# Megvii-CSG/MegReader

Measured on AMD Instinct MI355X. Metric: training images/sec, CRNN-CTC 32x128 crops, batch 256 per GPU, higher is better.
Workload: dtype bf16; 1 GPU; CRNN + 1D-CTC training step (BASELINE.json configs[1]): 32x128 crops, T=33, C=38, Adam; global_batch=256, per_gpu_batch=256, parallelism=dp1, launch=hipGraph replay

## Files before the change

megreader_amd/_lib.py:

```python
import ctypes
import os
import re

import torch

_HERE = os.path.dirname(os.path.abspath(__file__))
LIB_PATH = os.environ.get("MEGREADER_HIP_LIB") or os.path.join(_HERE, "csrc", "libmegreader_hip.so")
HEADER_PATH = os.path.join(os.path.dirname(_HERE), "include", "megreader_hip.h")

MR_F32 = 0
MR_BF16 = 1

_PARAM_TYPES = {"int": ctypes.c_int, "long long": ctypes.c_longlong, "float": ctypes.c_float, "double": ctypes.c_double,
                "hipStream_t": ctypes.c_void_p}
_RETURN_TYPES = {"int": ctypes.c_int, "long long": ctypes.c_longlong, "const char*": ctypes.c_char_p}


def _ctype(decl, context, array_ok=False):
    m = re.fullmatch(r"(.*?)(\w+)(?:\[(\d+)\])?", decl.strip(), re.S)
    base = " ".join(m.group(1).split()) if m else ""
    ctype = ctypes.c_void_p if "*" in base else _PARAM_TYPES.get(base)
    if ctype is None or (m.group(3) and not array_ok):
        raise TypeError("cannot bind %r in `%s`: no ctypes mapping for that type" % (decl.strip(), " ".join(context.split())))
    return m.group(2), ctype * int(m.group(3)) if m.group(3) else ctype, base == "hipStream_t"
# ... 19 lines not shown
    for stmt in filter(None, (s.strip() for s in text.split(";"))):
        if stmt == "}":
            continue
        m = re.fullmatch(r"(.*?)\b(mr_\w+)\s*\((.*)\)", stmt, re.S)
        ret = re.sub(r"\s*\*\s*", "*", " ".join(m.group(1).split())) if m else None
        if ret not in _RETURN_TYPES or m.group(2) in functions:
            raise TypeError("cannot bind `%s`: not a declaration `int | long long | const char* mr_name(...)`"
                            % " ".join(stmt.split()))
        params = [] if m.group(3).strip() in ("", "void") else [_ctype(p, stmt) for p in m.group(3).split(",")]
        functions[m.group(2)] = (_RETURN_TYPES[ret], [p[1] for p in params], bool(params) and params[-1][2])
    return functions, structs, defines


def _read_header(path):
    if not os.path.exists(path):
        raise RuntimeError("C ABI header not found at %s -- the ctypes binding is derived from it (there is no fallback table)"
                           % path)
    with open(path) as f:
        return parse_header(f.read())


FUNCTIONS, STRUCTS, _DEFINES = _read_header(HEADER_PATH)
ABI_VERSION = _DEFINES["MR_ABI_VERSION"]
TUNING_FIELDS = tuple(name for name, _ in STRUCTS["mr_tuning"] if name != "reserved")
_STREAMED = frozenset(name for name, (_, _, streamed) in FUNCTIONS.items() if streamed)

_lib = None


class Tuning(ctypes.Structure):
    _fields_ = STRUCTS["mr_tuning"]


def get_tuning():
    t = Tuning()
    if load().mr_tuning_get(ctypes.byref(t)) != 0:
        raise RuntimeError("mr_tuning_get failed: %s" % load().mr_last_error().decode())
    return {name: getattr(t, name) for name in TUNING_FIELDS}


def set_tuning(**fields):
    lib = load()
    t = Tuning()
    if lib.mr_tuning_get(ctypes.byref(t)) != 0:
        raise RuntimeError("mr_tuning_get failed: %s" % lib.mr_last_error().decode())
    old = {}
    for name, value in fields.items():
        if name not in TUNING_FIELDS:
            raise KeyError("mr_tuning has no field %r" % name)
        old[name] = getattr(t, name)
        setattr(t, name, int(value))
    if lib.mr_tuning_set(ctypes.byref(t)) != 0:
        raise RuntimeError("mr_tuning_set failed: %s" % lib.mr_last_error().decode())
    return old


def _install_setter_shims(lib):
    def one(field, clamp=None):
        def setter(value):
            value = int(value)
            if clamp is not None and not clamp(value):
                return get_tuning()[field]
            return set_tuning(**{field: value})[field]
        return setter
    lib.mr_set_nt_variant = one("nt_variant", lambda v: v in (1, 2))
    lib.mr_set_nt_deep = one("nt_deep", lambda v: 0 <= v <= 2)
    lib.mr_set_nt_big = one("nt_big", lambda v: -1 <= v <= 13)
    lib.mr_set_nt_p8 = one("nt_p8")
    lib.mr_set_gemm_skinny = lambda v: one("gemm_skinny")(1 if v else 0)
    lib.mr_set_tn_big = one("tn_big", lambda v: -1 <= v <= 2)
    lib.mr_set_tn_buf = one("tn_buf", lambda v: v in (0, 1))
    lib.mr_set_tn_taps = one("tn_taps", lambda v: v in (0, 1))
    lib.mr_set_tn_taps_group = one("tn_taps_group", lambda v: v >= 0)
    lib.mr_set_tn_group = one("tn_group", lambda v: v >= 0)
    lib.mr_set_tn_fin = one("tn_fin", lambda v: v in (0, 2))
    lib.mr_set_tn_taps_fin = one("tn_taps_fin", lambda v: 0 <= v <= 2)
    lib.mr_set_tn_taps_w8 = one("tn_taps_w8", lambda v: v in (0, 1))
    lib.mr_set_tn_model = lambda v: one("tn_model")(1 if v else 0)
    lib.mr_set_tn_splits = lambda v: one("tn_splits")(max(0, int(v)))
    lib.mr_set_bn_fused = one("bn_fused", lambda v: v in (0, 1))
    lib.mr_set_dcn_fused = lambda v: one("dcn_fused")(1 if v else 0)
    lib.mr_set_dcn_v1_bwd = lambda v: one("dcn_v1_bwd")(1 if v else 0)

    def set_lstm_persist(on):
        set_tuning(lstm_persist=int(on) if int(on) in (0, 1, 2) else 1)
        return 0
    lib.mr_set_lstm_persist = set_lstm_persist

    def set_lstm_variant(fwd_bn, bwd_bn):
        f = {}
        if fwd_bn >= 0:
            f["lstm_fwd_bn"] = fwd_bn
        if bwd_bn >= 0:
            f["lstm_bwd_bn"] = bwd_bn
        set_tuning(**f)
        return 0
    lib.mr_set_lstm_variant = set_lstm_variant

    def force_nt_tile(bm, bn):
        set_tuning(nt_force_bm=bm, nt_force_bn=bn if bm else 0)
        return 0
    lib.mr_force_nt_tile = force_nt_tile


def header_symbols():
    return sorted(FUNCTIONS)


def _bind(lib, functions, optional=False):
    for name, (restype, argtypes, _) in functions.items():
        if optional and not hasattr(lib, name):
            continue
        fn = getattr(lib, name)
        fn.restype, fn.argtypes = restype, argtypes


def load():
    global _lib
    if _lib is not None:
        return _lib
    if not os.path.exists(LIB_PATH):
        raise RuntimeError(
            "libmegreader_hip.so not found at %s -- build it with `python -c 'import __graft_entry__ as g; "
            "g.build()'` or `make -C megreader_amd/csrc` (there is no CPU fallback)" % LIB_PATH)
    lib = ctypes.CDLL(LIB_PATH)
    if lib.mr_abi_version() != ABI_VERSION:
        raise RuntimeError("%s implements C ABI version %d, this binding expects %d -- rebuild it (`make -C megreader_amd/csrc`)"
                           % (LIB_PATH, lib.mr_abi_version(), ABI_VERSION))
    _bind(lib, FUNCTIONS)
    _bind(lib, _read_header(os.path.join(os.path.dirname(HEADER_PATH), "megreader_hip_ablation.h"))[0], optional=True)
    _install_setter_shims(lib)
    _lib = lib
    if torch.cuda.is_available():
        if lib.mr_init() != 0:
            raise RuntimeError("mr_init failed: %s" % lib.mr_last_error().decode())
    elif lib.mr_init() != 0:
        err = lib.mr_last_error().decode()
        if "MEGREADER_TUNING" in err:
            raise RuntimeError("mr_init failed: %s" % err)
    return lib


def dtype_code(dtype):
    if dtype == torch.float32:
        return MR_F32
    if dtype == torch.bfloat16:
        return MR_BF16
    raise TypeError("megreader_amd kernels support float32 and bfloat16, got %s" % dtype)


def vec_of(dtype):
    return 4 if dtype == torch.float32 else 8


def stream_ptr():
    return torch.cuda.current_stream().cuda_stream


def ptr(t):
    return 0 if t is None else t.data_ptr()


class KernelTimer(object):

    def __init__(self, names, track_deferred=False):
        self.names = set(names)
# ... 97 lines not shown
```

megreader_amd/csrc/gemm_conv.hip:

```cpp
#include "igemm_core.h"
#include "igemm_p8.h"
#include "tn_taps.h"
#include "nt32.h"
#include "device.h"
#include "../../include/megreader_hip.h"

#include <algorithm>
#include <cmath>
#include <map>
#include <mutex>
#include <vector>

namespace mr {

static bool aligned16(const void* p) { return (((uintptr_t)p) & 15) == 0; }

#define g_nt_variant MR_TUNE(nt_variant)
#define g_nt_deep MR_TUNE(nt_deep)

struct BnbRequest { const void* x; const void* y; const float* mean; const float* rstd; };
struct NtEpilogue {
  const float* bias = nullptr;
  int relu = 0;
  const void* addend = nullptr;
// ... 87 lines not shown
  if constexpr (AMODE != 1) {
    if (g_nt_variant == 2 && nt_fits_buffer<T>(a, g, AMODE)) {
      const int grid = cdiv(cdiv(a.M - a.m_begin, BM), 8) * 8 * cdiv(a.N, BN);
      NtArgs a2 = a;
      a2.zero = zero_page();
      if (!a2.zero) { set_error("zero page allocation failed"); return MR_ERR_LAUNCH; }
      if constexpr (AMODE == 2) {
        if (o.bnb.x != nullptr) {
          EpiStoreB<T> eb;
          static_cast<EpiStore<T>&>(eb) = epi;
          eb.bnb_x = (const T*)o.bnb.x;
          eb.bnb_y = (const T*)o.bnb.y;
          eb.bnb_mean = o.bnb.mean;
          eb.bnb_rstd = o.bnb.rstd;
          return launch_nt_glds<T, BM, BN, AMODE, EpiStoreB<T>>(a2, g, eb, grid, tiles, stream);
        }
      }
      return launch_nt_glds<T, BM, BN, AMODE, EpiStore<T>>(a2, g, epi, grid, tiles, stream);
    }
  }
  if (a.m_begin != 0) { set_error("row-range launches need the direct-to-LDS NT kernel"); return MR_ERR_ARG; }
  if (o.stats) o.stats_missed = true;
  epi.stats = nullptr;
  hipLaunchKernelGGL((igemm_nt_kernel<T, BM, BN, AMODE, EpiStore<T>>), dim3(tiles), dim3(256), 0, stream, a, g,
                     epi);
  MR_CHECK_LAUNCH();
  return MR_OK;
}

#define g_big_mode MR_TUNE(nt_big)
#ifdef MR_ABLATION
static int g_tn_abl = 0;
#endif
#define g_tn_model MR_TUNE(tn_model)
#define g_tn_splits MR_TUNE(tn_splits)
#define g_tn_buf MR_TUNE(tn_buf)
#define g_tn_taps MR_TUNE(tn_taps)
#define g_tn_group MR_TUNE(tn_group)
#define g_tn_fin MR_TUNE(tn_fin)
#define g_tn_big MR_TUNE(tn_big)

static int nt_big_choice(int M, int N, int K) {
  if (g_big_mode < 0) return 0;
  if (g_big_mode > 0) return g_big_mode;
  if (N % 256 != 0 || K < MR_TUNE(nt_big_min_k)) return 0;
  const int cus = num_cus();
  const long long tiles = (long long)cdiv(M, 256) * (N / 256);
  const long long rounds = (tiles + cus - 1) / cus;
  const double util = (double)M * N / ((double)rounds * cus * 256 * 256);
  if (util >= 0.85) return 1;
  const long long tiles272 = (long long)cdiv(M, 272) * (N / 256);
  const long long rounds272 = (tiles272 + cus - 1) / cus;
  const double util272 = (double)M * N / ((double)rounds272 * cus * 272 * 256);
  if (util272 >= 0.85) {
    const int tiles_n = N / 256;
    double alt = 1e300;
    if (cus % tiles_n == 0) {
      const long long rows_per_round = (long long)(cus / tiles_n) * 256;
      const long long head = (M / rows_per_round) * rows_per_round;
      if (head > 0 && (M - head) * 8 <= M) alt = (double)(head / rows_per_round) * 256 + (head == M ? 0 : 57);
    }
    if ((double)rounds272 * 272 < alt) return 3;
  }
  return 0;
}

static long long nt_head_rows(int M, int N, int K) {
  if (g_big_mode != 0 || N % 256 != 0 || K < MR_TUNE(nt_big_min_k)) return 0;
  const int cus = num_cus();
  const int tiles_n = N / 256;
  if (cus % tiles_n != 0) return 0;
  const long long rows_per_round = (long long)(cus / tiles_n) * 256;
  const long long head = (M / rows_per_round) * rows_per_round;
  return (head > 0 && (M - head) * 8 <= M) ? head : 0;
}

template <typename T, int WM, int WN, int TM, int TN, int AMODE>
static int launch_nt_big(const NtArgs& a, const ConvGeom& g, void* C, long long ldc, NtEpilogue& o, hipStream_t stream) {
  constexpr int BM = WM * TM * 16, BN = WN * TN * 16;
  const EpiStore<T> epi = make_epi_store<T>(C, ldc, a.M, a.N, o);
  NtArgs a2 = a;
  a2.zero = zero_page();
  if (!a2.zero) { set_error("zero page allocation failed"); return MR_ERR_LAUNCH; }
  constexpr size_t lds = 2 * (size_t)(BM + BN) * 128;
  auto kern = igemm_nt_big_kernel<T, WM, WN, TM, TN, AMODE, EpiStore<T>>;
  if (const int rc = ensure_dynamic_lds(kern, lds)) return rc;
  const int tiles_m = cdiv(a.M - a.m_begin, BM), tiles_n = cdiv(a.N, BN);
  const int grid = cdiv(tiles_m, 8) * 8 * tiles_n;
  hipLaunchKernelGGL(kern, dim3(grid), dim3(64 * WM * WN), lds, stream, a2, g, epi);
  MR_CHECK_LAUNCH();
  return MR_OK;
}

#define g_use_p8 MR_TUNE(nt_p8)
template <typename T, int AMODE>
static int launch_nt_p8(const NtArgs& a, const ConvGeom& g, void* C, long long ldc, NtEpilogue& o, hipStream_t stream) {
  if constexpr (sizeof(T) != 2) {
    return launch_nt_big<T, 2, 4, 8, 4, AMODE>(a, g, C, ldc, o, stream);
  } else {
    if (!g_use_p8) return launch_nt_big<T, 2, 4, 8, 4, AMODE>(a, g, C, ldc, o, stream);
    const EpiStore<T> epi = make_epi_store<T>(C, ldc, a.M, a.N, o);
    NtArgs a2 = a;
    a2.zero = zero_page();
    if (!a2.zero) { set_error("zero page allocation failed"); return MR_ERR_LAUNCH; }
    constexpr size_t lds = 2 * (size_t)(256 + 256) * 128;
    const int tiles_m = cdiv(a.M - a.m_begin, 256), tiles_n = cdiv(a.N, 256);
    const int grid = cdiv(tiles_m, 8) * 8 * tiles_n;
#define MR_P8_LAUNCH(ABL_)                                                    \
  {                                                                           \
    auto kern = igemm_nt_p8_kernel<AMODE, EpiStore<T>, ABL_>;                 \
    if (const int rc = ensure_dynamic_lds(kern, lds)) return rc;              \
    hipLaunchKernelGGL(kern, dim3(grid), dim3(512), lds, stream, a2, g, epi); \
  }
#ifdef MR_ABLATION
    if (g_use_p8 == 2) MR_P8_LAUNCH(1)
    else if (g_use_p8 == 3) MR_P8_LAUNCH(2)
    else if (g_use_p8 == 4) MR_P8_LAUNCH(3)
    else
#endif
    MR_P8_LAUNCH(0)
#undef MR_P8_LAUNCH
    MR_CHECK_LAUNCH();
    return MR_OK;
  }
}

struct TileChoice { int bm, bn; };
static inline TileChoice forced_tile() { return TileChoice{MR_TUNE(nt_force_bm), MR_TUNE(nt_force_bn)}; }
static TileChoice nt_tile(int M, int N) {
  if (forced_tile().bm) return forced_tile();
  static const int bms[3] = {128, 96, 64};
  static const int bns[2] = {128, 64};
  auto eff = [](int bm, int bn) {
    if (bn == 128) return bm == 128 ? 1.0 : bm == 96 ? 0.90 : 0.85;
    return bm == 128 ? 0.60 : bm == 96 ? 0.60 : 0.55;
  };
  const int cus = num_cus();
  TileChoice best = {128, 128};
  double best_t = 1e300;
  for (int i = 0; i < 3; ++i)
    for (int j = 0; j < 2; ++j) {
      const int bm = bms[i], bn = bns[j];
      if (bn == 128 && N <= 64) continue;
      const long long tiles = (long long)cdiv(M, bm) * cdiv(N, bn);
      const int lds = 2 * (bm + bn) * 128;
      int per_cu = (160 * 1024) / lds;
      if (per_cu > 3) per_cu = 3;
      long long c = (tiles + cus - 1) / cus;
      if (c > per_cu) c = per_cu;
      const long long rounds = (tiles + cus * c - 1) / (cus * c);
      const double t = (double)rounds * c * bm * bn / eff(bm, bn);
      if (t < best_t) { best_t = t; best.bm = bm; best.bn = bn; }
    }
  return best;
}

static bool nt_use_288x128(int M, int N, int K) {
  if (g_big_mode != 0 || N % 128 != 0 || K < 2048) return false;
  const int cus = num_cus();
  const long long tiles = (long long)cdiv(M, 288) * (N / 128);
  const long long rounds = (tiles + cus - 1) / cus;
  const double util = (double)M * N / ((double)rounds * cus * 288 * 128);
  if (util < 0.85) return false;
  const TileChoice t = nt_tile(M, N);
  const long long t4 = (long long)cdiv(M, t.bm) * cdiv(N, t.bn);
  int per_cu = (160 * 1024) / (2 * (t.bm + t.bn) * 128);
// ... 378 lines not shown
        void* ws = nullptr;
        long long ws_bytes = 0;
        taps_get_workspace(&ws, &ws_bytes);
        int want = g_tn_group > 1 ? g_tn_group : 4;
        if (want > splits) want = splits;
        const long long need = TN_TICKETS * 4ll + (long long)tiles * splits * 65536;
        if (ws && need <= ws_bytes && need < (1ll << 31) && (long long)tiles * cdiv(splits, want) <= TN_TICKETS) {
          a.grp = want;
          a.ws = ws;
        }
      }
      const void* z = zero_page();
      if (!z) { set_error("zero page allocation failed"); return MR_ERR_LAUNCH; }
      const bool buf_ok = tn_fits_buffer(a, g, BMODE);
#ifdef MR_ABLATION
      if (g_tn_abl && buf_ok) {
#define MR_TN_ABL(V_) case V_: hipLaunchKernelGGL((igemm_tn_glds_kernel<BMODE, true, V_>), dim3(tiles * splits), \
                                                   dim3(256), 0, stream, a, g, z); break;
        switch (g_tn_abl) { MR_TN_ABL(1) MR_TN_ABL(2) MR_TN_ABL(3) MR_TN_ABL(4) MR_TN_ABL(8) MR_TN_ABL(15) default: break; }
#undef MR_TN_ABL
      } else
#endif
      if (g_tn_buf && buf_ok)
        hipLaunchKernelGGL((igemm_tn_glds_kernel<BMODE, true>), dim3(tiles * splits), dim3(256), 0, stream, a, g, z);
      else
        hipLaunchKernelGGL((igemm_tn_glds_kernel<BMODE, false>), dim3(tiles * splits), dim3(256), 0, stream, a, g, z);
      MR_CHECK_LAUNCH();
      if (a.fin == 2) {
        hipLaunchKernelGGL(tn_finalize_kernel, dim3(tiles * 16), dim3(256), 0, stream,
                           (const f32x4*)((const char*)a.ws + TN_TICKETS * 4), a.C, tiles, cdiv(a.NB, 128), splits, a.NA, a.NB,
                           a.ldc, a.row_perm_h);
        MR_CHECK_LAUNCH();
      }
      return MR_OK;
    }
  }
  hipLaunchKernelGGL((igemm_tn_kernel<T, BMODE>), dim3(tiles, 1, splits), dim3(256), 0, stream, a, g);
  MR_CHECK_LAUNCH();
  return MR_OK;
}

}

using namespace mr;

namespace mr {
bool gemm_nt_skinny(int dtype, const void* A, long long lda, const void* B, long long ldb, void* C, long long ldc,
                    const float* bias, int relu, int M, int N, int K, hipStream_t stream);
}

static int conv_pool_plan(int M, int N, int K, int Cin, int Ho, int Wo, int kh, int sh, int ph, int* tile_rows) {
  if (kh != sh || ph != 0 || Ho % kh != 0 || (Cin % 64) != 0 || g_nt_variant != 2) return 0;
  const int img = Ho * Wo, wrow = kh * Wo;
  auto fit = [&](int bm) {
    int t = (bm / wrow) * wrow;
    if (t <= 0) return 0;
    if (t >= img) t = (t / img) * img;
    else while (t > 0 && img % t != 0) t -= wrow;
    return t;
  };
  const int big = nt_big_choice(M, N, K);
  if (big == 1 || big == 3) {
    const int bm = big == 1 ? 256 : 272;
    const int t = fit(bm);
    if (t > 0 && N % 256 == 0 && t * 16 >= bm * 15) { *tile_rows = t; return big; }
  }
  const TileChoice tw = nt_tile(M, N);
  if (tw.bm == 128 && tw.bn == 128 && (MR_TUNE(nt_wide8) & 1) && N % 128 == 0) {
    const int t = fit(128);
    if (t == 128) { *tile_rows = t; return 8; }
  }
  return 0;
}

template <int WM, int WN, int TM, int TN>
static int launch_nt_pool(const NtArgs& a, const ConvGeom& g, const EpiPool<bf16_t>& epi, hipStream_t stream) {
  constexpr int BM = WM * TM * 16, BN = WN * TN * 16;
  constexpr size_t lds_stage = 2 * (size_t)(BM + BN) * 128, lds_tile = (size_t)BM * BN * 2;
  constexpr size_t lds = lds_stage > lds_tile ? lds_stage : lds_tile;
  auto kern = igemm_nt_big_kernel<bf16_t, WM, WN, TM, TN, 2, EpiPool<bf16_t>>;
  if (const int rc = ensure_dynamic_lds(kern, lds)) return rc;
  const int tiles_m = cdiv(a.M, a.tile_rows), tiles_n = cdiv(a.N, BN);
  const int grid = cdiv(tiles_m, 8) * 8 * tiles_n;
  hipLaunchKernelGGL(kern, dim3(grid), dim3(64 * WM * WN), lds, stream, a, g, epi);
  MR_CHECK_LAUNCH();
  return MR_OK;
}


extern "C" {

int mr_init(void) {
  const int rc = tuning_from_env();
  if (rc != MR_OK) return rc;
  if (!zero_page()) { set_error("mr_init: zero page allocation failed"); return MR_ERR_LAUNCH; }
  return MR_OK;
}

#ifdef MR_ABLATION
int mr_set_tn_abl(int mask) {
  const int old = g_tn_abl;
  g_tn_abl = mask;
  return old;
}
int mr_set_tn_taps_abl(int mask) { return taps_set_abl(mask); }
#endif

int mr_set_tn_taps_workspace(void* ws, long long bytes) {
  MR_CHECK_ARG((ws == nullptr) == (bytes == 0) && bytes >= 0 && (((uintptr_t)ws) & 15) == 0,
               "mr_set_tn_taps_workspace: bad workspace");
  taps_set_workspace(ws, bytes);
  return MR_OK;
}

int mr_tn_taps_would_run(int Nimg, int H, int W, int Cin, int ldx, int Cout, int lddy, int R, int S, int sh, int sw,
                         int ph, int pw, int dh, int dw, int Ho, int Wo) {
  return (g_tn_taps && g_nt_variant == 2 &&
          taps_eligible(Nimg, H, W, Cin, ldx, Cout, lddy, R, S, sh, sw, ph, pw, dh, dw, Ho, Wo,
                        (long long)Nimg * Ho * Wo * 8)) ? 1 : 0;
}

int mr_tn_taps_plan(int cus, int slabs, int n, const int* tiles, const int* chunks, int* launch, int* splits, int* cps,
                    double* cost) {
  const double c = tiles && chunks && launch && splits && cps ? taps_plan(cus, slabs, n, tiles, chunks, launch, splits, cps) : -1.0;
  if (c < 0.0) {
    set_error("mr_tn_taps_plan: need 1 <= n <= %d, cus > 0, tiles > 0, chunks > 0 and non-null arrays", TAPS_PLAN_MAX);
    return -1;
  }
  if (cost) *cost = c;
  int launches = 0;
  for (int i = 0; i < n; ++i) launches = std::max(launches, launch[i] + 1);
  return launches;
}

int mr_tn_group_plan(int cus, int n, const int* tiles, const int* steps, const int* modes, int* launch, int* splits, int* begin,
                     double* cost) {
  const double c = tiles && steps && modes && launch && splits && begin
                       ? tn_group_plan(cus, n, tiles, steps, modes, launch, splits, begin) : -1.0;
  if (c < 0.0) {
    set_error("mr_tn_group_plan: need 1 <= n <= %d, cus > 0, tiles > 0, steps > 0, modes 0 / 2 and non-null arrays", TN_PLAN_MAX);
    return -1;
  }
  if (cost) *cost = c;
  return *std::max_element(launch, launch + n) + 1;
}

int mr_tn_group_cost(int cus, int n, const int* tiles, const int* steps, const int* modes, const int* splits, double* cost) {
  bool ok = cus > 0 && n >= 1 && n <= TN_PLAN_MAX && tiles && steps && modes && splits && cost;
  for (int i = 0; ok && i < n; ++i)
    ok = tiles[i] > 0 && steps[i] > 0 && splits[i] > 0 && splits[i] <= steps[i] && (modes[i] == 0 || modes[i] == 2);
  MR_CHECK_ARG(ok, "mr_tn_group_cost: need 1 <= n <= %d, cus > 0, tiles > 0, 1 <= splits <= steps, modes 0 / 2", TN_PLAN_MAX);
  *cost = tn_launch_cost(cus, n, tiles, steps, modes, splits);
  return MR_OK;
}

int mr_tn_capacity(int kind) { return kind == 0 ? TN_GROUP_MAX : kind == 1 ? TAPS_PLAN_MAX : 0; }

int mr_nt_tile_code(int M, int N) {
  const TileChoice t = nt_tile(M, N);
  return t.bm * 1000 + t.bn;
}

int mr_nt_kernel_code(int dtype, int M, int N, int K, int cg) {
  if (dtype == MR_BF16 && g_nt_variant == 2 && !forced_tile().bm && (cg == 0 || cg % 64 == 0)) {
    const int big = nt_big_choice(M, N, K);
    if (big == 1) return 256256;
    if (big == 2) return 288256;
// ... 281 lines not shown
```

megreader_amd/csrc/igemm_core.h:

```cpp
#pragma once
#include "common.h"
#include <type_traits>

namespace mr {

struct ConvGeom {
  int Hg, Wg, Cg, ldg;
  int Hm, Wm;
  int R, S, sh, sw, ph, pw, dh, dw;
  int mode;
};

__device__ __forceinline__ bool conv_src(const ConvGeom& g, int hm, int wm, int r, int s, int& hi, int& wi) {
  if (g.mode == 1) {
    hi = hm * g.sh - g.ph + r * g.dh;
    wi = wm * g.sw - g.pw + s * g.dw;
  } else {
    int hn = hm + g.ph - r * g.dh;
    int wn = wm + g.pw - s * g.dw;
    if (hn < 0 || wn < 0) return false;
    if (g.sh == 1 && g.sw == 1) {
      hi = hn;
      wi = wn;
    } else {
      hi = hn / g.sh;
      wi = wn / g.sw;
      if (hi * g.sh != hn || wi * g.sw != wn) return false;
    }
  }
  return (unsigned)hi < (unsigned)g.Hg && (unsigned)wi < (unsigned)g.Wg;
}

template <typename T> struct Mma;
template <> struct Mma<bf16_t> {
  typedef bf16x8 Frag;
  static __device__ __forceinline__ void run(f32x4& acc, const Frag& a, const Frag& b) {
    acc = __builtin_amdgcn_mfma_f32_16x16x32_bf16(a, b, acc, 0, 0, 0);
  }
};
template <> struct Mma<float> {
  typedef f32x4 Frag;
  static __device__ __forceinline__ void run(f32x4& acc, const Frag& a, const Frag& b) {
#pragma unroll
    for (int j = 0; j < 4; ++j) acc = __builtin_amdgcn_mfma_f32_16x16x4f32(a[j], b[j], acc, 0, 0, 0);
  }
};

struct NtArgs {
  const void* A;
  const void* B;
  int M, N, K;
  long long lda;
  int ldb;
  const void* zero;
  int m_begin = 0;
  int ksplit = 1;
  void* ws = nullptr;
  int tile_rows = 0;
};
constexpr int NT_SPLIT_TICKETS = 4096;

__device__ __forceinline__ uint4 ldg16(const void* p) { return *(const uint4*)p; }

template <typename Epi> struct EpiHasStats { static constexpr bool value = false; };
template <typename Epi> struct EpiIsPool { static constexpr bool value = false; };
__device__ __forceinline__ float row16_sum(float v) {
#define MR_ROW_ROR(V, N) __builtin_bit_cast(float, __builtin_amdgcn_update_dpp(0, __builtin_bit_cast(int, V), 0x120 + (N), 0xf, 0xf, false))
  v += MR_ROW_ROR(v, 8);
  v += MR_ROW_ROR(v, 4);
  v += MR_ROW_ROR(v, 2);
  v += MR_ROW_ROR(v, 1);
#undef MR_ROW_ROR
  return v;
}
template <typename T, int CNT> struct EpiColStats {
  float s[4 * CNT], q[4 * CNT];
  __device__ __forceinline__ void init() {
#pragma unroll
    for (int e = 0; e < 4 * CNT; ++e) s[e] = q[e] = 0.f;
  }
  template <typename Epi> __device__ __forceinline__ void add(const Epi& epi, int m, int n, const f32x4* v) {
    if (m >= epi.M) return;
    if constexpr (Epi::kBnb) {
      const long long row = (long long)m * epi.ldc + n;
#pragma unroll
      for (int i = 0; i < CNT; ++i)
#pragma unroll
        for (int j = 0; j < 4; ++j) {
          const int c = 4 * i + j;
          if (n + c < epi.N) {
            float t = v[i][j];
            if (epi.addend) t += to_f32(epi.addend[row + c]);
            t = to_f32(from_f32<T>(t));
            if (epi.bnb_y && !(to_f32(epi.bnb_y[row + c]) > 0.f)) t = 0.f;
            s[c] += t;
            q[c] += t * to_f32(epi.bnb_x[row + c]);
          }
        }
    } else {
#pragma unroll
      for (int i = 0; i < CNT; ++i)
#pragma unroll
        for (int j = 0; j < 4; ++j) {
          float t = v[i][j];
          if (epi.bias && n + 4 * i + j < epi.N) t += epi.bias[n + 4 * i + j];
          t = to_f32(from_f32<T>(t));
          s[4 * i + j] += t;
          q[4 * i + j] += t * t;
        }
    }
  }
  template <typename Epi> __device__ __forceinline__ double q_out(const Epi& epi, int c, float sv, float qv) const {
    if constexpr (Epi::kBnb) return ((double)qv - (double)epi.bnb_mean[c] * (double)sv) * (double)epi.bnb_rstd[c];
    else return (double)qv;
  }
  template <typename Epi> __device__ __forceinline__ void flush(const Epi& epi, int n, int l15) {
#pragma unroll
    for (int e = 0; e < 4 * CNT; ++e) {
      s[e] = row16_sum(s[e]);
      q[e] = row16_sum(q[e]);
    }
    double* dst = epi.stats + (size_t)(blockIdx.x % epi.stats_ncopy) * 2 * epi.N;
    if constexpr (CNT == 4) {
      float sv = s[0], qv = q[0];
#pragma unroll
      for (int e = 1; e < 16; ++e) {
        sv = l15 == e ? s[e] : sv;
        qv = l15 == e ? q[e] : qv;
      }
      if (n + l15 < epi.N) {
        atomicAdd(dst + n + l15, (double)sv);
        atomicAdd(dst + epi.N + n + l15, q_out(epi, n + l15, sv, qv));
      }
    } else if constexpr (CNT == 2) {
      const int c = l15 & 7;
      float sv = s[0], qv = q[0];
#pragma unroll
      for (int e = 1; e < 8; ++e) {
        sv = c == e ? s[e] : sv;
        qv = c == e ? q[e] : qv;
      }
// ... 879 lines not shown
  EpiColStats<T, TN> cst;
  bool with_stats = false;
  if constexpr (EpiHasStats<Epi>::value) with_stats = epi.stats != nullptr;
  if (with_stats) cst.init();
#pragma unroll
  for (int j = 0; j < TM; ++j) {
    f32x4 run[TN];
#pragma unroll
    for (int i = 0; i < TN; ++i) {
      if constexpr (WIDE) run[i] = (f32x4){(float)tot[i][j][0], (float)tot[i][j][1], (float)tot[i][j][2], (float)tot[i][j][3]};
      else run[i] = acc[i][j];
    }
    if constexpr (EpiHasStats<Epi>::value)
      if (with_stats) cst.add(epi, m0 + wm_ * WTM + j * 16 + l15, n0 + wn_ * WTN + lg * (4 * TN), run);
    epi.template store_run<TN>(m0 + wm_ * WTM + j * 16 + l15, n0 + wn_ * WTN + lg * (4 * TN), run);
  }
  if constexpr (EpiHasStats<Epi>::value)
    if (with_stats) cst.flush(epi, n0 + wn_ * WTN + lg * (4 * TN), l15);
}

template <typename T, int WM, int WN, int TM, int TN, int AMODE, typename Epi>
__global__ __launch_bounds__(64 * WM * WN) void igemm_nt_big_kernel(NtArgs a, ConvGeom g, Epi epi) {
  constexpr int VEC = VecOf<T>::N;
  constexpr int BK = 8 * VEC;
  constexpr int NW = WM * WN;
  constexpr int WTM = TM * 16, WTN = TN * 16, BM = WM * WTM, BN = WN * WTN;
  constexpr int AG = BM / 8, BG = BN / 8;
  constexpr int AI = (AG + NW - 1) / NW, BI = (BG + NW - 1) / NW;
  constexpr int TILE_VECS = (BM + BN) * 8;
  typedef typename Mma<T>::Frag Frag;
  static_assert(AMODE == 0 || AMODE == 2, "big-tile kernel: dense or fast conv gather only");

  extern __shared__ uint4 smem_big[];
  uint4* smem = smem_big;

  const int tid = threadIdx.x;
  const int wave = __builtin_amdgcn_readfirstlane(tid >> 6);
  const int lane = tid & 63;
  const int trows = a.tile_rows > 0 ? a.tile_rows : BM;
  const int tiles_n = (a.N + BN - 1) / BN, tiles_m = (a.M - a.m_begin + trows - 1) / trows;
  const int xcd = blockIdx.x & 7, slot = blockIdx.x >> 3;
  const int tile_m = (slot / tiles_n) * 8 + xcd, tile_n = slot % tiles_n;
  if (tile_m >= tiles_m) return;
  const int m0 = a.m_begin + tile_m * trows, n0 = tile_n * BN;
  const int lrow = lane >> 3, lpc = lane & 7;

  const T* __restrict__ A = (const T*)a.A;
  const T* __restrict__ B = (const T*)a.B;
  (void)a.zero;
  constexpr int ESH = sizeof(T) == 2 ? 1 : 2;
  const rsrc_t rsA = make_rsrc(A), rsB = make_rsrc(B);

  auto kc_of = [&](int gi) { return (lpc ^ (((gi * 8 + lrow) >> 1) & 7)) * VEC; };
  int a_off[AI];
  unsigned a_mask[AI];
#pragma unroll
  for (int i = 0; i < AI; ++i) {
    const int gi = wave + i * NW;
    const int m = m0 + gi * 8 + lrow;
    a_mask[i] = 0;
    a_off[i] = 0;
    if (gi < AG && gi * 8 + lrow < trows) {
      if (AMODE == 0) {
        a_off[i] = (int)((long long)m * a.lda + kc_of(gi));
        a_mask[i] = m < a.M ? 1u : 0u;
      } else if (m < a.M) {
        const int wm = m % g.Wm;
        const int t = m / g.Wm;
        const int hm = t % g.Hm;
        const int ni = t / g.Hm;
        const int bh = g.mode == 1 ? hm * g.sh - g.ph : hm + g.ph;
        const int bw = g.mode == 1 ? wm * g.sw - g.pw : wm + g.pw;
        a_off[i] = (int)((long long)ni * g.Hg * g.Wg * g.ldg + ((long long)bh * g.Wg + bw) * g.ldg + kc_of(gi));
        unsigned msk = 0;
        for (int r = 0; r < g.R; ++r)
          for (int s2 = 0; s2 < g.S; ++s2) {
            int hi, wi;
            if (conv_src(g, hm, wm, r, s2, hi, wi)) msk |= 1u << (r * g.S + s2);
          }
        a_mask[i] = msk;
      }
    }
  }
  int b_off[BI];
  unsigned b_okmask = 0;
#pragma unroll
  for (int i = 0; i < BI; ++i) {
    const int gi = wave + i * NW;
    const int row = gi * 8 + lrow;
    const int rb = row % WTN;
    const int n = n0 + (row - rb) + ((rb >> 2) & 3) * (4 * TN) + (rb >> 4) * 4 + (rb & 3);
    if (gi < BG && n < a.N) b_okmask |= 1u << i;
    b_off[i] = (int)((long long)n * a.ldb + kc_of(gi));
  }

  const int sgn = g.mode == 1 ? 1 : -1;
  const bool k_exact = (a.K % BK) == 0;
  int s_tap = 0, s_r = 0, s_s = 0, s_c0 = 0;

  auto stage = [&](uint4* sA, int k0) {
    uint4* sB = sA + BM * 8;
    if (AMODE == 0) {
#pragma unroll
      for (int i = 0; i < AI; ++i) {
        const int gi = wave + i * NW;
        if (AG % NW == 0 || gi < AG) {
          const bool ok = a_mask[i] && (k_exact || k0 + kc_of(gi) < a.K);
          glds16_buf(rsA, ok, a_off[i] + k0, ESH, sA + gi * 64);
        }
      }
    } else {
      const int koff = sgn * ((s_r * g.dh * g.Wg + s_s * g.dw) * g.ldg) + s_c0;
      const unsigned bit = 1u << s_tap;
#pragma unroll
      for (int i = 0; i < AI; ++i) {
        const int gi = wave + i * NW;
        if (AG % NW == 0 || gi < AG) glds16_buf(rsA, a_mask[i] & bit, a_off[i] + koff, ESH, sA + gi * 64);
      }
      s_c0 += BK;
      if (s_c0 >= g.Cg) {
        s_c0 = 0;
        ++s_tap;
        if (++s_s == g.S) { s_s = 0; ++s_r; }
      }
    }
#pragma unroll
    for (int i = 0; i < BI; ++i) {
      const int gi = wave + i * NW;
      if (BG % NW == 0 || gi < BG) {
        const bool ok = ((b_okmask >> i) & 1u) && (k_exact || k0 + kc_of(gi) < a.K);
        glds16_buf(rsB, ok, b_off[i] + k0, ESH, sB + gi * 64);
      }
    }
  };

  const int wm_ = wave % WM, wn_ = wave / WM;
  const int l15 = lane & 15, lg = lane >> 4;
  const int xsw = (l15 >> 1) & 7;
  const int fa_base = (wm_ * WTM + l15) * 8 + (lg ^ xsw);
  const int fb_base = BM * 8 + (wn_ * WTN + l15) * 8 + (lg ^ xsw);

  f32x4 acc[TN][TM];
#pragma unroll
  for (int i = 0; i < TN; ++i)
#pragma unroll
    for (int j = 0; j < TM; ++j) acc[i][j] = (f32x4){0.f, 0.f, 0.f, 0.f};

  auto compute = [&](const uint4* st) {
#pragma unroll
    for (int ks = 0; ks < 2; ++ks) {
      const uint4* sa = st + (ks ? (fa_base ^ 4) : fa_base);
      const uint4* sb = st + (ks ? (fb_base ^ 4) : fb_base);
      Frag fb[TN];
#pragma unroll
      for (int i = 0; i < TN; ++i) fb[i] = *(const Frag*)&sb[i * 128];
      Frag fa = *(const Frag*)&sa[0];
#pragma unroll
      for (int j = 0; j < TM; ++j) {
        Frag nxt = fa;
        if (j + 1 < TM) nxt = *(const Frag*)&sa[(j + 1) * 128];
#pragma unroll
        for (int i = 0; i < TN; ++i) Mma<T>::run(acc[i][j], fb[i], fa);
        fa = nxt;
      }
    }
  };

  const int nk = (a.K + BK - 1) / BK;
  uint4* st0 = smem;
  uint4* st1 = smem + TILE_VECS;
  if (nk > 0) stage(st0, 0);
  int t = 0;
  for (; t + 1 < nk; t += 2) {
    __syncthreads();
    stage(st1, (t + 1) * BK);
    compute(st0);
    __syncthreads();
    if (t + 2 < nk) stage(st0, (t + 2) * BK);
    compute(st1);
  }
  if (t < nk) {
    __syncthreads();
    compute(st0);
  }

  if constexpr (EpiIsPool<Epi>::value) {
    static_assert(sizeof(T) == 2, "pooled epilogue: bf16 only");
    constexpr int CH = BN / 8;
    static_assert((CH & (CH - 1)) == 0 && (4 * TN) % 8 == 0, "pooled epilogue: tile width / lane run in whole 16-byte chunks");
    __syncthreads();
    auto tile_to_lds = [&](auto bias_tag, auto relu_tag) {
      constexpr bool BIAS = decltype(bias_tag)::value, RELU = decltype(relu_tag)::value;
      const int nl = n0 + wn_ * WTN + lg * (4 * TN);
      float bv[4 * TN];
      if constexpr (BIAS) {
#pragma unroll
        for (int e = 0; e < 4 * TN; ++e) bv[e] = nl + e < epi.N ? epi.bias[nl + e] : 0.f;
      }
#pragma unroll
      for (int j = 0; j < TM; ++j) {
        const int r = wm_ * WTM + j * 16 + l15;
#pragma unroll
        for (int q = 0; q < TN / 2; ++q) {
          T o[8];
#pragma unroll
          for (int e = 0; e < 8; ++e) {
            float t = acc[2 * q + e / 4][j][e % 4];
            if constexpr (BIAS) t += bv[q * 8 + e];
            if constexpr (RELU) t = fmaxf(t, 0.f);
            o[e] = from_f32<T>(t);
          }
          const int c = (wn_ * WTN + lg * (4 * TN)) / 8 + q;
          smem[r * CH + (c ^ (r & (CH - 1)))] = *(const uint4*)o;
        }
      }
    };
    if (epi.bias != nullptr) {
      if (epi.relu) tile_to_lds(std::true_type{}, std::true_type{});
      else tile_to_lds(std::true_type{}, std::false_type{});
    } else {
      if (epi.relu) tile_to_lds(std::false_type{}, std::true_type{});
      else tile_to_lds(std::false_type{}, std::false_type{});
    }
    __syncthreads();
    const int img_rows = trows / epi.Wo;
    const int prows = img_rows / epi.kh;
    const int row0 = m0 / epi.Wo;
    constexpr int PSTEP = 64 * NW / CH;
    const int c = tid % CH;
    int pix = tid / CH;
    int pr = pix / epi.PWo, pwi = pix - pr * epi.PWo;
    int nimg = (row0 + pr * epi.kh) / epi.Ho, h = (row0 + pr * epi.kh) - nimg * epi.Ho;
    const bool col_ok = n0 + c * 8 < epi.N;
    auto pool_one = [&](auto kh_tag, auto kw_tag) {
      constexpr int KH = decltype(kh_tag)::value, KW = decltype(kw_tag)::value;
      const int kh = KH ? KH : epi.kh, kw = KW ? KW : epi.kw;
      for (; pr < prows; ) {
        if (nimg < epi.Nimg && col_ok) {
          float best[8];
          unsigned char bi[8] = {0, 0, 0, 0, 0, 0, 0, 0};
#pragma unroll
          for (int e = 0; e < 8; ++e) best[e] = -INFINITY;
          bool first = true;
#pragma unroll
          for (int i = 0; i < (KH ? KH : 1); ++i)
            for (int i2 = 0; i2 < (KH ? 1 : kh); ++i2) {
              const int ii = KH ? i : i2;
#pragma unroll
              for (int jx = 0; jx < (KW ? KW : 1); ++jx)
                for (int j2 = 0; j2 < (KW ? 1 : kw); ++j2) {
                  const int jj = KW ? jx : j2;
                  const int w = pwi * epi.sw - epi.pw + jj;
                  if ((unsigned)w >= (unsigned)epi.Wo) continue;
                  const int r = (pr * kh + ii) * epi.Wo + w;
                  const uint4 v = smem[r * CH + (c ^ (r & (CH - 1)))];
                  const T* pv = (const T*)&v;
#pragma unroll
                  for (int e = 0; e < 8; ++e) {
                    const float f = to_f32(pv[e]);
                    if (first || f > best[e] || f != f) { best[e] = f; bi[e] = (unsigned char)(ii * kw + jj); }
                  }
                  first = false;
                }
            }
          T o[8];
#pragma unroll
// ... 1013 lines not shown
```

megreader_amd/csrc/tuning.hip:

```cpp
#include <climits>
#include <cstdlib>
#include <cstring>
#include <mutex>

#include "common.h"
#include "tuning.h"

namespace mr {

#define MR_TUNING_DEFAULTS                                                                                              \
  {  2,  1,  0,  0,  0,  0,  1, \
     0,  1,  1,  0,  0,  0,  0,     \
     0,  1,  0,  1,  1,  0,            \
     32,  1,  1,  1,  0,  512,  10000,  1,  1,  1,  7,  1,  0,  0,  1,  1,  1, {0} }

mr_tuning g_tuning = MR_TUNING_DEFAULTS;
static const mr_tuning k_defaults = MR_TUNING_DEFAULTS;
static std::mutex g_tuning_mutex;

struct Field {
  const char* name;
  size_t offset;
  int lo, hi;
};
#define MR_F(f, lo, hi) {#f, offsetof(mr_tuning, f), lo, hi}
static const Field k_fields[] = {
    MR_F(nt_variant, 1, 2), MR_F(nt_deep, 0, 2), MR_F(nt_big, -1, 13),
#ifdef MR_ABLATION
    MR_F(nt_p8, 0, 4),
#else
    MR_F(nt_p8, 0, 1),
#endif
    MR_F(nt_force_bm, 0, 128), MR_F(nt_force_bn, 0, 128), MR_F(gemm_skinny, 0, 1), MR_F(tn_big, -1, 2), MR_F(tn_buf, 0, 1),
    MR_F(tn_taps, 0, 1), MR_F(tn_taps_group, 0, 1 << 20), MR_F(tn_group, 0, 1 << 20), MR_F(tn_fin, 0, 2),
    MR_F(tn_taps_fin, 0, 2), MR_F(tn_taps_w8, 0, 1), MR_F(tn_model, 0, 1), MR_F(tn_splits, 0, 1 << 20), MR_F(bn_fused, 0, 1),
    MR_F(lstm_persist, 0, 2), MR_F(lstm_fwd_bn, 0, 64), MR_F(lstm_bwd_bn, 0, 64), MR_F(dcn_fused, 0, 1),
    MR_F(dcn_v1_bwd, 0, 1), MR_F(bn_onepass, 0, 1), MR_F(skinny_depth, 0, 8), MR_F(nt_big_min_k, 32, 1 << 20), MR_F(tn_taps_min_p, 0, 1 << 30), MR_F(tn_defer, 0, 1), MR_F(pool_fixed, 0, 1), MR_F(ctc_linear, 0, 1), MR_F(nt_wide8, 0, 63), MR_F(nt_ksplit, 0, 8), MR_F(nt_m32, 0, 5), MR_F(nt_m32_opt, 0, 99), MR_F(dcn_gcol, 0, 1), MR_F(dcn_col_fwd, 0, 1), MR_F(decode_persist, 0, 2)};
#undef MR_F

static const char* check(const mr_tuning& t) {
  for (const Field& f : k_fields) {
    const int v = *(const int*)((const char*)&t + f.offset);
    if (v < f.lo || v > f.hi) return f.name;
  }
  if (t.tn_fin == 1) return "tn_fin";
  if (t.nt_force_bm != 0 && !((t.nt_force_bm == 128 || t.nt_force_bm == 96 || t.nt_force_bm == 64) &&
                              (t.nt_force_bn == 128 || t.nt_force_bn == 64)))
    return "nt_force_bm / nt_force_bn";
  if (!(t.skinny_depth == 0 || t.skinny_depth == 4 || t.skinny_depth == 8)) return "skinny_depth";
  if (!(t.lstm_fwd_bn == 0 || t.lstm_fwd_bn == 32 || t.lstm_fwd_bn == 64)) return "lstm_fwd_bn";
  if (!(t.lstm_bwd_bn == 0 || t.lstm_bwd_bn == 16 || t.lstm_bwd_bn == 32 || t.lstm_bwd_bn == 64)) return "lstm_bwd_bn";
  return nullptr;
}

static void store(const mr_tuning& t) {
  for (const Field& f : k_fields)
    __atomic_store_n((int*)((char*)&g_tuning + f.offset), *(const int*)((const char*)&t + f.offset), __ATOMIC_RELAXED);
}

int tuning_from_env() {
  static bool done = false;
  std::lock_guard<std::mutex> lock(g_tuning_mutex);
  if (done) return MR_OK;
  done = true;
  const char* env = std::getenv("MEGREADER_TUNING");
  if (!env || !*env) return MR_OK;
  mr_tuning t = g_tuning;
  char buf[1024];
  std::strncpy(buf, env, sizeof(buf) - 1);
  buf[sizeof(buf) - 1] = 0;
  for (char* tok = std::strtok(buf, ",; "); tok; tok = std::strtok(nullptr, ",; ")) {
    char* eq = std::strchr(tok, '=');
    if (!eq) { set_error("MEGREADER_TUNING: '%s' is not name=value", tok); return MR_ERR_ARG; }
    *eq = 0;
    bool found = false;
    for (const Field& f : k_fields)
      if (!std::strcmp(f.name, tok)) {
        *(int*)((char*)&t + f.offset) = std::atoi(eq + 1);
        found = true;
      }
    if (!found) { set_error("MEGREADER_TUNING: unknown field '%s'", tok); return MR_ERR_ARG; }
  }
  if (const char* bad = check(t)) { set_error("MEGREADER_TUNING: value of '%s' out of range", bad); return MR_ERR_ARG; }
  store(t);
  return MR_OK;
}

}

using namespace mr;

extern "C" {

int mr_tuning_get(mr_tuning* out) {
  MR_CHECK_ARG(out != nullptr, "mr_tuning_get: null");
  std::lock_guard<std::mutex> lock(g_tuning_mutex);
  *out = g_tuning;
  return MR_OK;
}

int mr_tuning_defaults(mr_tuning* out) {
  MR_CHECK_ARG(out != nullptr, "mr_tuning_defaults: null");
  *out = k_defaults;
  return MR_OK;
}

int mr_tuning_set(const mr_tuning* in) {
  MR_CHECK_ARG(in != nullptr, "mr_tuning_set: null");
  if (const char* bad = check(*in)) {
    set_error("mr_tuning_set: value of '%s' out of range", bad);
    return MR_ERR_ARG;
  }
  std::lock_guard<std::mutex> lock(g_tuning_mutex);
  store(*in);
  return MR_OK;
}

}
```

Baseline: 112,600 images/s.

## Skip MFMA work for padded conv taps in implicit-GEMM NT kernel

```diff
diff --git a/megreader_amd/_lib.py b/megreader_amd/_lib.py
--- a/megreader_amd/_lib.py
+++ b/megreader_amd/_lib.py
@@ -125,6 +125,17 @@
     lib.mr_set_dcn_fused = lambda v: one("dcn_fused")(1 if v else 0)
     lib.mr_set_dcn_v1_bwd = lambda v: one("dcn_v1_bwd")(1 if v else 0)
 
+    def set_nt_pad_skip(on):
+        t = Tuning()
+        if lib.mr_tuning_get(ctypes.byref(t)) != 0:
+            raise RuntimeError("mr_tuning_get failed: %s" % lib.mr_last_error().decode())
+        old = 0 if t.reserved[0] else 1
+        t.reserved[0] = 0 if int(on) else 1
+        if lib.mr_tuning_set(ctypes.byref(t)) != 0:
+            raise RuntimeError("mr_tuning_set failed: %s" % lib.mr_last_error().decode())
+        return old
+    lib.mr_set_nt_pad_skip = set_nt_pad_skip
+
     def set_lstm_persist(on):
         set_tuning(lstm_persist=int(on) if int(on) in (0, 1, 2) else 1)
         return 0
diff --git a/megreader_amd/csrc/gemm_conv.hip b/megreader_amd/csrc/gemm_conv.hip
--- a/megreader_amd/csrc/gemm_conv.hip
+++ b/megreader_amd/csrc/gemm_conv.hip
@@ -193,6 +193,7 @@
   NtArgs a2 = a;
   a2.zero = zero_page();
   if (!a2.zero) { set_error("zero page allocation failed"); return MR_ERR_LAUNCH; }
+  a2.pad_skip = MR_TUNE(reserved[0]) == 0;
   constexpr size_t lds = 2 * (size_t)(BM + BN) * 128;
   auto kern = igemm_nt_big_kernel<T, WM, WN, TM, TN, AMODE, EpiStore<T>>;
   if (const int rc = ensure_dynamic_lds(kern, lds)) return rc;
@@ -737,7 +738,9 @@
   if (const int rc = ensure_dynamic_lds(kern, lds)) return rc;
   const int tiles_m = cdiv(a.M, a.tile_rows), tiles_n = cdiv(a.N, BN);
   const int grid = cdiv(tiles_m, 8) * 8 * tiles_n;
-  hipLaunchKernelGGL(kern, dim3(grid), dim3(64 * WM * WN), lds, stream, a, g, epi);
+  NtArgs a2 = a;
+  a2.pad_skip = MR_TUNE(reserved[0]) == 0;
+  hipLaunchKernelGGL(kern, dim3(grid), dim3(64 * WM * WN), lds, stream, a2, g, epi);
   MR_CHECK_LAUNCH();
   return MR_OK;
 }
diff --git a/megreader_amd/csrc/igemm_core.h b/megreader_amd/csrc/igemm_core.h
--- a/megreader_amd/csrc/igemm_core.h
+++ b/megreader_amd/csrc/igemm_core.h
@@ -57,6 +57,7 @@
   int ksplit = 1;
   void* ws = nullptr;
   int tile_rows = 0;
+  int pad_skip = 0;
 };
 constexpr int NT_SPLIT_TICKETS = 4096;
 
@@ -1102,6 +1103,22 @@
       }
     }
   }
+  constexpr bool PAD_SKIP = AMODE == 2 && WM == 1 && NW == 8;
+  bool pad_skip = false;
+  if constexpr (PAD_SKIP) {
+    pad_skip = a.pad_skip != 0 && g.R * g.S > 1 && g.R * g.S <= 9;
+    if (pad_skip) {
+      unsigned* gmask = (unsigned*)(smem + (BM + BN) * 8);
+#pragma unroll
+      for (int i = 0; i < AI; ++i) {
+        const int gi = wave + i * NW;
+        unsigned u = 0;
+#pragma unroll
+        for (int tp = 0; tp < 9; ++tp) u |= (__builtin_amdgcn_ballot_w64(((a_mask[i] >> tp) & 1u) != 0) != 0 ? 1u : 0u) << tp;
+        if ((AG % NW == 0 || gi < AG) && lane == 0) gmask[gi] = u;
+      }
+    }
+  }
   int b_off[BI];
   unsigned b_okmask = 0;
 #pragma unroll
@@ -1160,13 +1177,36 @@
   const int fa_base = (wm_ * WTM + l15) * 8 + (lg ^ xsw);
   const int fb_base = BM * 8 + (wn_ * WTN + l15) * 8 + (lg ^ xsw);
 
+  constexpr int NBP = (TM + 2) / 3;
+  unsigned blk_taps[NBP];
+#pragma unroll
+  for (int j = 0; j < NBP; ++j) blk_taps[j] = 0u;
+  unsigned blk_all = 0xFFFFFFFFu, tap_full = 0u;
+  int c_tap = 0, c_c0 = 0;
+  if constexpr (PAD_SKIP) {
+    const int taps = g.R * g.S;
+    if (pad_skip) {
+      const unsigned* gmask = (const unsigned*)(smem + TILE_VECS);
+      tap_full = (1u << taps) - 1u;
+      __syncthreads();
+#pragma unroll
+      for (int j = 0; j < TM; ++j) {
+        const uint2 v = *(const uint2*)&gmask[(wm_ * TM + j) * 2];
+        const unsigned m = (unsigned)__builtin_amdgcn_readfirstlane((int)(v.x | v.y));
+        blk_taps[j / 3] |= m << (9 * (j % 3));
+        blk_all &= m;
+      }
+    }
+  }
+
   f32x4 acc[TN][TM];
 #pragma unroll
   for (int i = 0; i < TN; ++i)
 #pragma unroll
     for (int j = 0; j < TM; ++j) acc[i][j] = (f32x4){0.f, 0.f, 0.f, 0.f};
 
-  auto compute = [&](const uint4* st) {
+  auto compute_body = [&](const uint4* st, auto skip_tag, unsigned tapbit) {
+    constexpr bool SKIP = decltype(skip_tag)::value;
 #pragma unroll
     for (int ks = 0; ks < 2; ++ks) {
       const uint4* sa = st + (ks ? (fa_base ^ 4) : fa_base);
@@ -1179,29 +1219,56 @@
       for (int j = 0; j < TM; ++j) {
         Frag nxt = fa;
         if (j + 1 < TM) nxt = *(const Frag*)&sa[(j + 1) * 128];
-#pragma unroll
-        for (int i = 0; i < TN; ++i) Mma<T>::run(acc[i][j], fb[i], fa);
+        unsigned live = 1u;
+        if constexpr (SKIP) {
+          live = blk_taps[j / 3] & (tapbit << (9 * (j % 3)));
+          asm volatile("" : "+s"(live));
+        }
+        if (live != 0) {
+#pragma unroll
+          for (int i = 0; i < TN; ++i) Mma<T>::run(acc[i][j], fb[i], fa);
+        }
         fa = nxt;
       }
     }
   };
-
   const int nk = (a.K + BK - 1) / BK;
   uint4* st0 = smem;
   uint4* st1 = smem + TILE_VECS;
-  if (nk > 0) stage(st0, 0);
-  int t = 0;
-  for (; t + 1 < nk; t += 2) {
-    __syncthreads();
-    stage(st1, (t + 1) * BK);
-    compute(st0);
-    __syncthreads();
-    if (t + 2 < nk) stage(st0, (t + 2) * BK);
-    compute(st1);
-  }
-  if (t < nk) {
-    __syncthreads();
-    compute(st0);
+  auto main_loop = [&](auto skip_tag) {
+    constexpr bool SKIP = decltype(skip_tag)::value;
+    auto compute = [&](const uint4* st) {
+      unsigned tapbit = 0u;
+      if constexpr (SKIP) {
+        tapbit = 1u << c_tap;
+        c_c0 += BK;
+        if (c_c0 >= g.Cg) {
+          c_c0 = 0;
+          ++c_tap;
+        }
+      }
+      compute_body(st, skip_tag, tapbit);
+    };
+    if (nk > 0) stage(st0, 0);
+    int t = 0;
+    for (; t + 1 < nk; t += 2) {
+      __syncthreads();
+      stage(st1, (t + 1) * BK);
+      compute(st0);
+      __syncthreads();
+      if (t + 2 < nk) stage(st0, (t + 2) * BK);
+      compute(st1);
+    }
+    if (t < nk) {
+      __syncthreads();
+      compute(st0);
+    }
+  };
+  if constexpr (PAD_SKIP) {
+    if ((blk_all & tap_full) != tap_full) main_loop(std::true_type{});
+    else main_loop(std::false_type{});
+  } else {
+    main_loop(std::false_type{});
   }
 
   if constexpr (EpiIsPool<Epi>::value) {
diff --git a/megreader_amd/csrc/tuning.hip b/megreader_amd/csrc/tuning.hip
--- a/megreader_amd/csrc/tuning.hip
+++ b/megreader_amd/csrc/tuning.hip
@@ -35,7 +35,8 @@
     MR_F(tn_taps, 0, 1), MR_F(tn_taps_group, 0, 1 << 20), MR_F(tn_group, 0, 1 << 20), MR_F(tn_fin, 0, 2),
     MR_F(tn_taps_fin, 0, 2), MR_F(tn_taps_w8, 0, 1), MR_F(tn_model, 0, 1), MR_F(tn_splits, 0, 1 << 20), MR_F(bn_fused, 0, 1),
     MR_F(lstm_persist, 0, 2), MR_F(lstm_fwd_bn, 0, 64), MR_F(lstm_bwd_bn, 0, 64), MR_F(dcn_fused, 0, 1),
-    MR_F(dcn_v1_bwd, 0, 1), MR_F(bn_onepass, 0, 1), MR_F(skinny_depth, 0, 8), MR_F(nt_big_min_k, 32, 1 << 20), MR_F(tn_taps_min_p, 0, 1 << 30), MR_F(tn_defer, 0, 1), MR_F(pool_fixed, 0, 1), MR_F(ctc_linear, 0, 1), MR_F(nt_wide8, 0, 63), MR_F(nt_ksplit, 0, 8), MR_F(nt_m32, 0, 5), MR_F(nt_m32_opt, 0, 99), MR_F(dcn_gcol, 0, 1), MR_F(dcn_col_fwd, 0, 1), MR_F(decode_persist, 0, 2)};
+    MR_F(dcn_v1_bwd, 0, 1), MR_F(bn_onepass, 0, 1), MR_F(skinny_depth, 0, 8), MR_F(nt_big_min_k, 32, 1 << 20), MR_F(tn_taps_min_p, 0, 1 << 30), MR_F(tn_defer, 0, 1), MR_F(pool_fixed, 0, 1), MR_F(ctc_linear, 0, 1), MR_F(nt_wide8, 0, 63), MR_F(nt_ksplit, 0, 8), MR_F(nt_m32, 0, 5), MR_F(nt_m32_opt, 0, 99), MR_F(dcn_gcol, 0, 1), MR_F(dcn_col_fwd, 0, 1), MR_F(decode_persist, 0, 2),
+    {"nt_pad_skip_off", offsetof(mr_tuning, reserved), 0, 1}};
 #undef MR_F
 
 static const char* check(const mr_tuning& t) {
```

Result: no change. 113,100 images/s (median of 6 runs) (+0.5%).
